# yvette256/nerfstudio-thermal

Measured on AMD Instinct MI355X. Metric: train rays/sec (4096-ray batch, 96 samples/ray), higher is better.
Workload: dtype f32; 1 GPU; thermal-nerfacto density_mode=shared train step (pixel sampling+raygen+fwd+losses+bwd+allreduce+Adam), 4096 rays/GPU, 256/96 proposal + 48 field samples, hash 16x2^19x2 + 2x(5x2^17x2), 8 cameras (4 RGB + 4 thermal); rays_per_gpu=4096, parallelism=dp1, grad_scaler=device-side (optim.DeviceGradScaler)

## Files before the change

nerfstudio-thermal_amd/csrc/tn_field.hip:

```cpp
#include "tn_common.h"
#include "tn_field_dpos.h"
#include <stdlib.h>

typedef float f32x16 __attribute__((ext_vector_type(16)));
typedef float v4f_t __attribute__((ext_vector_type(4)));
#ifndef FRAG_NT
#define FRAG_NT 1
#endif

#define TILE 32
#define FRAG 64

__host__ __device__ __forceinline__ constexpr int RROW(int r, int h) { return (r & 3) + 8 * (r >> 2) + 4 * h; }

struct LayerGeom { int mo, ti; };
__host__ __device__ __forceinline__ constexpr int layer_mo(int l) { return (l == 0 || l == 2 || l == 3) ? 2 : 1; }
__host__ __device__ __forceinline__ constexpr int layer_ti(int l) { return l == 0 ? 1 : 2; }
__host__ __device__ __forceinline__ constexpr int layer_frags(int l) { return layer_mo(l) * layer_ti(l) * 16; }
__host__ __device__ __forceinline__ constexpr int fwd_off(int l) {
  int o = 0;
  for (int i = 0; i < l; ++i) o += layer_frags(i) * FRAG;
  return o;
}
#define PACK_FWD_FLOATS (fwd_off(5))
// ... 116 lines not shown
  int64_t bytes;
};
static inline FieldWs ws_layout(void* base, int64_t P, int training) {
  FieldWs w;
  char* p = reinterpret_cast<char*>(base);
  int64_t off = 0;
  auto take = [&](int64_t floats) {
    float* r = reinterpret_cast<float*>(p + off);
    off += ((floats * 4 + 255) / 256) * 256;
    return r;
  };
  const int64_t PT = tn_cdiv(P, 32) * 32;
  w.PT = PT;
  w.pack = take(PACK_REGION_FLOATS);
  w.pos = take(P * 4);
  w.enc = take(PT * 32);
  w.sel = take(P);
  w.sh = take(P * 16);
  if (training) {
    w.h1 = take(PT * 64); w.hin = take(PT * 16); w.hh1 = take(PT * 64); w.hh2 = take(PT * 64); w.y = take(P * 4);
    w.g_enc = take(P * 32);
    w.jac = take(PT * 96);
    w.cam_bias = take((int64_t)FIELD_MAX_IMAGES * 64 + 64);
    w.scatter = take(tn_scatter_scratch_bytes(P, TN_MAX_LEVELS) / 4);
  } else {
    w.h1 = w.hin = w.hh1 = w.hh2 = w.y = w.g_enc = w.jac = w.cam_bias = nullptr;
    w.scatter = nullptr;
  }
  w.bytes = off;
  return w;
}
extern "C" int64_t tn_field_workspace_bytes(int64_t num_points, int32_t training) {
  if (num_points < 0) return TN_EINVAL;
  return ws_layout(nullptr, num_points, training).bytes;
}

__device__ __forceinline__ void sh16(float dx, float dy, float dz, float* c);
template <bool PACK>
__global__ void __launch_bounds__(256) k_field_prep(FieldK f, float* __restrict__ pack, const float* __restrict__ origins,
                                                    const float* __restrict__ directions, const float* __restrict__ e_bins, int64_t N, int S,
                                                    float4* __restrict__ pos, float* __restrict__ sel, float* __restrict__ shtab,
                                                    float4* __restrict__ zero, int64_t zero_n4, float4* __restrict__ cam_bias, int cam_bias_n4) {
  int bid = blockIdx.x, nblk = gridDim.x;
  if (PACK) {
    const int pkb = PACK_BLOCKS + ((f.num_images < FIELD_MAX_IMAGES ? f.num_images : FIELD_MAX_IMAGES) * 64 + 255) / 256 + PACK_BF_WORDS / 256;
    if (bid < pkb) { field_pack_body(f, pack, bid * 256 + threadIdx.x); return; }
    bid -= pkb; nblk -= pkb;
  }
  for (int64_t i = bid * (int64_t)blockDim.x + threadIdx.x; i < zero_n4; i += (int64_t)nblk * blockDim.x) zero[i] = make_float4(0.f, 0.f, 0.f, 0.f);
  for (int64_t i = bid * (int64_t)blockDim.x + threadIdx.x; i < cam_bias_n4; i += (int64_t)nblk * blockDim.x) cam_bias[i] = make_float4(0.f, 0.f, 0.f, 0.f);
  if (cam_bias_n4 > 0 && bid == 0 && threadIdx.x == 0) cam_bias[FIELD_MAX_IMAGES * 16] = make_float4(0.f, 0.f, 0.f, 0.f);
  const int64_t P = N * (int64_t)S;
  for (int64_t p = bid * (int64_t)blockDim.x + threadIdx.x; p < P; p += (int64_t)nblk * blockDim.x) {
    const int64_t ray = tn_div_index(p, S, P);
    const int s = (int)(p - ray * S);
    const float* o = origins + ray * 3;
    const float* d = directions + ray * 3;
    const float* eb = e_bins + ray * (S + 1) + s;
    const Contracted c = tn_contract(o[0], o[1], o[2], d[0], d[1], d[2], eb[0], eb[1]);
    const float m = c.sel ? 1.0f : 0.0f;
    pos[p] = make_float4(c.px, c.py, c.pz, m);
    sel[p] = m;
    if (s == 0) {
      float sh[16];
      sh16(d[0], d[1], d[2], sh);
#pragma unroll
      for (int hh = 0; hh < 2; ++hh)
#pragma unroll
        for (int r = 0; r < 8; ++r) shtab[ray * 16 + hh * 8 + r] = sh[(r & 3) + 8 * (r >> 2) + 4 * hh];
    }
  }
}

#ifndef ENC_PER
#define ENC_PER 4
#endif
#define ENC_CHUNK (128 * ENC_PER)
#define ENC_MAX_ITEMS 2
static_assert(TN_MAX_LEVELS <= 8 * ENC_MAX_ITEMS, "encode plan");
struct EncSched {
  int16_t level[8][ENC_MAX_ITEMS];
  int32_t first[8][ENC_MAX_ITEMS + 1];
  int32_t c0[8][ENC_MAX_ITEMS];
  int32_t blocks_per_xcd;
};
static EncSched make_enc_sched(const TnGrid& g, int64_t P) {
  EncSched sc;
  const int chunks = (int)tn_cdiv(P, ENC_CHUNK);
  int mx = 0;
  for (int x = 0; x < 8; ++x) {
    int n = 0;
    sc.first[x][0] = 0;
    for (int l = x; l < g.num_levels && n < ENC_MAX_ITEMS; l += 8) {
      sc.level[x][n] = (int16_t)l;
      sc.c0[x][n] = 0;
      sc.first[x][n + 1] = sc.first[x][n] + chunks;
      ++n;
    }
    for (int i = n; i < ENC_MAX_ITEMS; ++i) { sc.level[x][i] = -1; sc.c0[x][i] = 0; sc.first[x][i + 1] = sc.first[x][n]; }
    mx = sc.first[x][n] > mx ? sc.first[x][n] : mx;
  }
  sc.blocks_per_xcd = mx;
  return sc;
}
template <bool JAC>
__global__ void __launch_bounds__(256) k_field_encode_xcd(GridK g, EncSched sc, const float4* __restrict__ pos, int64_t P, int64_t PT,
                                                          float* __restrict__ enc, float* __restrict__ jac) {
  const int x = blockIdx.x & 7, q = blockIdx.x >> 3;
  int item = 0;
#pragma unroll
  for (int i = 1; i < ENC_MAX_ITEMS; ++i) item += (q >= sc.first[x][i]) ? 1 : 0;
  if (q >= sc.first[x][ENC_MAX_ITEMS]) return;
  const int l = sc.level[x][item];
  const int chunk = sc.c0[x][item] + (q - sc.first[x][item]);
  const float res = g.res[l];
  const uint32_t off = (uint32_t)l * g.tsize;
  const int side = threadIdx.x & 1;
  const int64_t base = (int64_t)chunk * ENC_CHUNK + (threadIdx.x >> 1);
  float2 fv[ENC_PER][4];
  float ox[ENC_PER], oy[ENC_PER], oz[ENC_PER];
#pragma unroll
  for (int u = 0; u < ENC_PER; ++u) {
    int64_t p = base + u * 128;
    if (p >= P) p = P - 1;
    const float4 c = pos[p];
    const float sx = c.x * res, sy = c.y * res, sz = c.z * res;
    const float fxf = floorf(sx), fyf = floorf(sy), fzf = floorf(sz);
    const uint32_t xi = side ? (uint32_t)(int)fxf : (uint32_t)(int)ceilf(sx);
    const uint32_t hcy = (uint32_t)(int)ceilf(sy) * TN_PRIME_Y, hfy = (uint32_t)(int)fyf * TN_PRIME_Y;
    const uint32_t hcz = (uint32_t)(int)ceilf(sz) * TN_PRIME_Z, hfz = (uint32_t)(int)fzf * TN_PRIME_Z;
    ox[u] = sx - fxf; oy[u] = sy - fyf; oz[u] = sz - fzf;
    fv[u][0] = tn_table_entry(g.table, ((xi ^ hcy ^ hcz) & g.mask) + off);
    fv[u][1] = tn_table_entry(g.table, ((xi ^ hfy ^ hcz) & g.mask) + off);
    fv[u][2] = tn_table_entry(g.table, ((xi ^ hcy ^ hfz) & g.mask) + off);
    fv[u][3] = tn_table_entry(g.table, ((xi ^ hfy ^ hfz) & g.mask) + off);
  }
#pragma unroll
  for (int u = 0; u < ENC_PER; ++u) {
    const int64_t p = base + u * 128;
    const float ux = 1.0f - ox[u], uy = 1.0f - oy[u], uz = 1.0f - oz[u];
    const float wk = side ? ux : ox[u], wr = side ? ox[u] : ux;
    float t[4], dk[4];
#pragma unroll
    for (int k = 0; k < 4; ++k) {
      const float keep = side ? fv[u][k].y : fv[u][k].x, send = side ? fv[u][k].x : fv[u][k].y;
      const float recv = __int_as_float(__builtin_amdgcn_mov_dpp(__float_as_int(send), 0xB1, 0xF, 0xF, true));
      t[k] = keep * wk + recv * wr;
      if (JAC) dk[k] = side ? recv - keep : keep - recv;
    }
    const float f0312 = t[0] * oy[u] + t[1] * uy, f4756 = t[2] * oy[u] + t[3] * uy;
    const float r = f0312 * oz[u] + f4756 * uz;
    if (p >= P) continue;
    enc[((int64_t)l * PT + p) * 2 + side] = r;
    if (JAC) {
      const float dx = (dk[0] * oy[u] + dk[1] * uy) * oz[u] + (dk[2] * oy[u] + dk[3] * uy) * uz;
      const float dy = (t[0] - t[1]) * oz[u] + (t[2] - t[3]) * uz;
      const float dz = f0312 - f4756;
      float* jp = jac + ((int64_t)l * 3 * PT + p) * 2 + side;
      __builtin_nontemporal_store(dx * res, jp);
      __builtin_nontemporal_store(dy * res, jp + 2 * PT);
      __builtin_nontemporal_store(dz * res, jp + 4 * PT);
    }
  }
}

__global__ void __launch_bounds__(256) k_field_emb_finish(float* __restrict__ cam_bias, uint32_t* __restrict__ counter, const float* __restrict__ hw0,
                                                          const float* __restrict__ emb, float* __restrict__ gemb, float* __restrict__ ghw0, int num_images) {
  __shared__ float sums[64];
  __shared__ int flag;
  emb_finish_jobs(cam_bias, counter, hw0, emb, gemb, ghw0, num_images, sums, &flag, blockIdx.x, gridDim.x);
}

__global__ void __launch_bounds__(256) k_field_dpos(DposArgs a) {
  __shared__ float emb_sums[64];
  __shared__ int emb_flag;
  field_dpos_body(a, blockIdx.x, gridDim.x, emb_sums, &emb_flag);
}

__device__ __forceinline__ void sh16(float dx, float dy, float dz, float* c) {
  float x = (dx + 1.0f) / 2.0f, y = (dy + 1.0f) / 2.0f, z = (dz + 1.0f) / 2.0f;
  float xx = x * x, yy = y * y, zz = z * z;
  c[0] = 0.28209479177387814f;
  c[1] = 0.4886025119029199f * y;
  c[2] = 0.4886025119029199f * z;
  c[3] = 0.4886025119029199f * x;
  c[4] = 1.0925484305920792f * x * y;
  c[5] = 1.0925484305920792f * y * z;
  c[6] = 0.9461746957575601f * zz - 0.31539156525251999f;
  c[7] = 1.0925484305920792f * x * z;
  c[8] = 0.5462742152960396f * (xx - yy);
  c[9] = 0.5900435899266435f * y * (3.0f * xx - yy);
  c[10] = 2.890611442640554f * x * y * z;
  c[11] = 0.4570457994644658f * y * (5.0f * zz - 1.0f);
  c[12] = 0.3731763325901154f * z * (5.0f * zz - 3.0f);
  c[13] = 0.4570457994644658f * x * (5.0f * zz - 1.0f);
  c[14] = 1.445305721320277f * z * (xx - yy);
  c[15] = 0.5900435899266435f * x * (xx - 3.0f * yy);
}

#define MFMA(a, b, c) __builtin_amdgcn_mfma_f32_32x32x2f32((a), (b), (c), 0, 0, 0)
typedef __bf16 bf16x8 __attribute__((ext_vector_type(8)));
#define MFMAB(a, b, c) __builtin_amdgcn_mfma_f32_32x32x16_bf16((a), (b), (c), 0, 0, 0)
template <int S8>
__device__ __forceinline__ void bf_split8(const f32x16& v, bf16x8& hi, bf16x8& lo) {
#pragma unroll
  for (int q = 0; q < 8; ++q) {
    const float x = v[8 * S8 + q];
    const __bf16 hq = (__bf16)x;
    hi[q] = hq;
    lo[q] = (__bf16)(x - (float)hq);
  }
}
template <int T>
__device__ __forceinline__ void bf3_tile_fwd(const float* __restrict__ frags, int lane, const f32x16& x, f32x16& o0, f32x16& o1) {
  bf16x8 bh, bl;
#define BF_FRAG(m, s, part) (*reinterpret_cast<const bf16x8*>(frags + ((((((m) * 2 + T) * 2 + (s)) * 2 + (part))) << 8) + (lane << 2)))
#define BF_KSTEP(s)                                                                       \
  {                                                                                       \
    const bf16x8 a0h = BF_FRAG(0, s, 0), a0l = BF_FRAG(0, s, 1), a1h = BF_FRAG(1, s, 0), a1l = BF_FRAG(1, s, 1); \
    o0 = MFMAB(a0l, bh, o0); o1 = MFMAB(a1l, bh, o1);                                     \
    o0 = MFMAB(a0h, bl, o0); o1 = MFMAB(a1h, bl, o1);                                     \
    o0 = MFMAB(a0h, bh, o0); o1 = MFMAB(a1h, bh, o1);                                     \
  }
  bf_split8<0>(x, bh, bl);
  BF_KSTEP(0)
  bf_split8<1>(x, bh, bl);
  BF_KSTEP(1)
#undef BF_KSTEP
#undef BF_FRAG
}

__device__ __forceinline__ f32x16 bias_tile(const float* __restrict__ lds_bias, int layer, int m, int h) {
  f32x16 v;
#pragma unroll
  for (int r = 0; r < 16; ++r) v[r] = lds_bias[layer * 64 + 32 * m + RROW(r, h)];
  return v;
}
__device__ __forceinline__ f32x16 relu16(f32x16 v) {
#pragma unroll
  for (int r = 0; r < 16; ++r) v[r] = fmaxf(v[r], 0.0f);
  return v;
}
__device__ __forceinline__ void store_tile(float* __restrict__ base, int64_t p, int ld, int m, int h, const f32x16& v) {
#pragma unroll
  for (int g = 0; g < 4; ++g)
    *reinterpret_cast<float4*>(base + p * ld + 32 * m + 8 * g + 4 * h) = make_float4(v[4 * g], v[4 * g + 1], v[4 * g + 2], v[4 * g + 3]);
}
__device__ __forceinline__ f32x16 load_tile(const float* __restrict__ base, int64_t p, int ld, int m, int h) {
  f32x16 v;
#pragma unroll
  for (int g = 0; g < 4; ++g) {
    float4 t = *reinterpret_cast<const float4*>(base + p * ld + 32 * m + 8 * g + 4 * h);
    v[4 * g] = t.x; v[4 * g + 1] = t.y; v[4 * g + 2] = t.z; v[4 * g + 3] = t.w;
  }
  return v;
}

__device__ __forceinline__ void store_frag(float* __restrict__ base, int64_t tile, int M, int m, int lane, const f32x16& v) {
  v4f_t* b = reinterpret_cast<v4f_t*>(base) + ((tile * M + m) * 4) * 64 + lane;
#pragma unroll
  for (int g = 0; g < 4; ++g) {
    const v4f_t t = {v[4 * g], v[4 * g + 1], v[4 * g + 2], v[4 * g + 3]};
    if (FRAG_NT) __builtin_nontemporal_store(t, b + g * 64); else b[g * 64] = t;
  }
}
__device__ __forceinline__ f32x16 load_frag(const float* __restrict__ base, int64_t tile, int M, int m, int lane) {
  const v4f_t* b = reinterpret_cast<const v4f_t*>(base) + ((tile * M + m) * 4) * 64 + lane;
  f32x16 v;
#pragma unroll
  for (int g = 0; g < 4; ++g) {
    const v4f_t t = FRAG_NT ? __builtin_nontemporal_load(b + g * 64) : b[g * 64];
    v[4 * g] = t.x; v[4 * g + 1] = t.y; v[4 * g + 2] = t.z; v[4 * g + 3] = t.w;
  }
  return v;
}
__device__ __forceinline__ void store_bo(float* __restrict__ base, int64_t tile, int lane, const f32x16& bo) {
  v4f_t* b = reinterpret_cast<v4f_t*>(base) + tile * 128 + lane;
  const v4f_t t0 = {bo[0], bo[1], bo[2], bo[3]}, t1 = {bo[4], bo[5], bo[6], bo[7]};
  if (FRAG_NT) { __builtin_nontemporal_store(t0, b); __builtin_nontemporal_store(t1, b + 64); }
  else { b[0] = t0; b[64] = t1; }
}
__device__ __forceinline__ int64_t hin_logit_index(int64_t tile, int j) { return (tile * 128 + j) * 4; }
__device__ __forceinline__ f32x16 load_enc_lm(const float* __restrict__ enc, int64_t PT, int64_t pc, int h, int L) {
  f32x16 v;
  const uint32_t voff = (uint32_t)(((int64_t)(2 * h) * PT + pc) * 8);
  const char* e = reinterpret_cast<const char*>(enc);
#pragma unroll
  for (int q = 0; q < 4; ++q) {
    const int l0 = 4 * q + 2 * h;
    const char* b0 = e + (int64_t)(4 * q) * PT * 8;
    const float2 a = l0 < L ? *reinterpret_cast<const float2*>(b0 + voff) : make_float2(0.f, 0.f);
    const float2 b = l0 + 1 < L ? *reinterpret_cast<const float2*>(b0 + PT * 8 + voff) : make_float2(0.f, 0.f);
    v[4 * q] = a.x; v[4 * q + 1] = a.y; v[4 * q + 2] = b.x; v[4 * q + 3] = b.y;
  }
  return v;
}

#ifndef FWD_THREADS
#define FWD_THREADS 256
#endif
#ifndef FWD_ABLATE
#define FWD_ABLATE 0
#endif
#ifndef FWD_HEAD2_MFMA
#define FWD_HEAD2_MFMA 0
#endif
#ifndef FWD_EMB_MFMA
#define FWD_EMB_MFMA 0
#endif
template <bool TRAIN, bool BF3>
__global__ void __launch_bounds__(FWD_THREADS, FWD_THREADS / 128) k_field_mlp_fwd(const float* __restrict__ pack, const float* __restrict__ encs, int L,
                                                            int64_t PT, const float* __restrict__ sels, const float* __restrict__ shtab,
                                                            const int64_t* __restrict__ cam_idx, const float* __restrict__ emb, int num_images,
                                                            int use_cam_emb, int64_t N, int S, int C, float* __restrict__ density,
                                                            float* __restrict__ rgb, float* __restrict__ density_pre, float* __restrict__ h1s,
                                                            float* __restrict__ hins, float* __restrict__ hh1s, float* __restrict__ hh2s,
                                                            float* __restrict__ ys) {
  extern __shared__ __attribute__((aligned(16))) float lds[];
  const int lane = threadIdx.x & 63, j = lane & 31, h = lane >> 5;
  const int64_t P = N * (int64_t)S;
  const int64_t ntiles = tn_cdiv(P, TILE);
  const int64_t wave = (int64_t)blockIdx.x * (blockDim.x >> 6) + (threadIdx.x >> 6);
  const int64_t nwaves = (int64_t)gridDim.x * (blockDim.x >> 6);
  f32x16 nin;
  if (wave < ntiles) {
    const int64_t p0 = wave * TILE + j;
    nin = (FWD_ABLATE & 4) ? f32x16{0.1f, 0.2f, 0.3f, 0.4f, 0.5f, 0.6f, 0.7f, 0.8f, 0.1f, 0.2f, 0.3f, 0.4f, 0.5f, 0.6f, 0.7f, 0.8f} : load_enc_lm(encs, PT, p0 < P ? p0 : P - 1, h, L);
  }
  for (int i = threadIdx.x * 4; i < PACK_FWD_TOTAL; i += blockDim.x * 4) {
    const float* src = (BF3 && i >= fwd_off(2) && i < fwd_off(4)) ? pack + PACK_BF_OFF + (i - fwd_off(2)) : pack + i;
    *reinterpret_cast<float4*>(lds + i) = *reinterpret_cast<const float4*>(src);
  }
  __syncthreads();
  const float* lbias = lds + PACK_BIAS_OFF;
#define AF(layer, m, t, r) lds[fwd_off(layer) + ((((m) * layer_ti(layer) + (t)) * 16 + (r)) << 6) + lane]
  for (int64_t tile = wave; tile < ntiles; tile += nwaves) {
    const int64_t p = tile * TILE + j;
    const bool valid = p < P;
    const int64_t pc = valid ? p : P - 1;
    const int64_t ray = tn_div_index(pc, S, P);
    const float sl = sels[pc];
    const f32x16 in0 = nin;
    f32x16 a0 = bias_tile(lbias, 0, 0, h), a1 = bias_tile(lbias, 0, 1, h);
#pragma unroll
    for (int r = 0; r < 16; ++r) {
      a0 = MFMA(AF(0, 0, 0, r), in0[r], a0);
      a1 = MFMA(AF(0, 1, 0, r), in0[r], a1);
    }
    {
      const int64_t tn = tile + nwaves < ntiles ? tile + nwaves : tile;
      const int64_t pn = tn * TILE + j;
      if (!(FWD_ABLATE & 4)) nin = load_enc_lm(encs, PT, pn < P ? pn : P - 1, h, L);
    }
    __builtin_amdgcn_sched_barrier(0);
    a0 = relu16(a0); a1 = relu16(a1);
    if (TRAIN && !(FWD_ABLATE & 1)) { store_frag(h1s, tile, 2, 0, lane, a0); store_frag(h1s, tile, 2, 1, lane, a1); }
    f32x16 bo = bias_tile(lbias, 1, 0, h);
#pragma unroll
    for (int r = 0; r < 16; ++r) bo = MFMA(AF(1, 0, 0, r), a0[r], bo);
#pragma unroll
    for (int r = 0; r < 16; ++r) bo = MFMA(AF(1, 0, 1, r), a1[r], bo);
    __builtin_amdgcn_sched_barrier(0);
    if (valid && h == 0 && !(FWD_ABLATE & 16)) {
      float pre = bo[0];
      density[p] = expf(pre) * sl;
      if (density_pre) density_pre[p] = pre;
    }
    if (TRAIN && !(FWD_ABLATE & 1)) store_bo(hins, tile, lane, bo);
    f32x16 hi0, hi1;
    {
      const float4 zz = make_float4(0.1f, 0.2f, 0.3f, 0.4f);
      const float4 s0 = (FWD_ABLATE & 2) ? zz : *reinterpret_cast<const float4*>(shtab + ray * 16 + h * 8), s1 = (FWD_ABLATE & 2) ? zz : *reinterpret_cast<const float4*>(shtab + ray * 16 + h * 8 + 4);
      hi0[0] = s0.x; hi0[1] = s0.y; hi0[2] = s0.z; hi0[3] = s0.w; hi0[4] = s1.x; hi0[5] = s1.y; hi0[6] = s1.z; hi0[7] = s1.w;
    }
#pragma unroll
    for (int r = 0; r < 8; ++r) hi0[8 + r] = bo[r];
    f32x16 c0 = bias_tile(lbias, 2, 0, h), c1 = bias_tile(lbias, 2, 1, h);
    constexpr bool CAMHEAD = TRAIN && !FWD_EMB_MFMA;
    if (CAMHEAD && !(FWD_ABLATE & 2)) {
      int64_t cam = cam_idx[ray];
      if (cam < 0 || cam >= num_images) cam = 0;
      const float* chp = pack + PACK_CAMHEAD_OFF + cam * 64 + 4 * h;
#pragma unroll
      for (int gq = 0; gq < 4; ++gq) {
        const float4 u0 = *reinterpret_cast<const float4*>(chp + 8 * gq), u1 = *reinterpret_cast<const float4*>(chp + 32 + 8 * gq);
        c0[4 * gq] += u0.x; c0[4 * gq + 1] += u0.y; c0[4 * gq + 2] += u0.z; c0[4 * gq + 3] += u0.w;
        c1[4 * gq] += u1.x; c1[4 * gq + 1] += u1.y; c1[4 * gq + 2] += u1.z; c1[4 * gq + 3] += u1.w;
      }
    } else if (!CAMHEAD) {
      const float* ebp;
      if (use_cam_emb) {
        int64_t cam = cam_idx[ray];
        if (cam < 0 || cam >= num_images) cam = 0;
        ebp = emb + cam * 32;
      } else {
        ebp = lds + PACK_MEANEMB_OFF;
      }
#pragma unroll
      for (int gq = 0; gq < 4; ++gq)
#pragma unroll
        for (int q = 0; q < 4; ++q) hi1[4 * gq + q] = ebp[8 * gq + 4 * h + q];
    }
    __builtin_amdgcn_sched_barrier(0);
    if (BF3) {
      bf3_tile_fwd<0>(lds + fwd_off(2), lane, hi0, c0, c1);
      if (!CAMHEAD && !(FWD_ABLATE & 2)) bf3_tile_fwd<1>(lds + fwd_off(2), lane, hi1, c0, c1);
    } else {
#pragma unroll
      for (int r = 0; r < 16; ++r) { c0 = MFMA(AF(2, 0, 0, r), hi0[r], c0); c1 = MFMA(AF(2, 1, 0, r), hi0[r], c1); }
      if (!CAMHEAD && !(FWD_ABLATE & 2)) {
#pragma unroll
        for (int r = 0; r < 16; ++r) { c0 = MFMA(AF(2, 0, 1, r), hi1[r], c0); c1 = MFMA(AF(2, 1, 1, r), hi1[r], c1); }
      }
    }
    __builtin_amdgcn_sched_barrier(0);
    c0 = relu16(c0); c1 = relu16(c1);
    if (TRAIN && !(FWD_ABLATE & 1)) { store_frag(hh1s, tile, 2, 0, lane, c0); store_frag(hh1s, tile, 2, 1, lane, c1); }
    f32x16 d0 = bias_tile(lbias, 3, 0, h), d1 = bias_tile(lbias, 3, 1, h);
    if (BF3) {
      bf3_tile_fwd<0>(lds + fwd_off(2) + PACK_BF_LAYER_WORDS, lane, c0, d0, d1);
      bf3_tile_fwd<1>(lds + fwd_off(2) + PACK_BF_LAYER_WORDS, lane, c1, d0, d1);
    } else {
#pragma unroll
      for (int r = 0; r < 16; ++r) { d0 = MFMA(AF(3, 0, 0, r), c0[r], d0); d1 = MFMA(AF(3, 1, 0, r), c0[r], d1); }
#pragma unroll
      for (int r = 0; r < 16; ++r) { d0 = MFMA(AF(3, 0, 1, r), c1[r], d0); d1 = MFMA(AF(3, 1, 1, r), c1[r], d1); }
    }
    __builtin_amdgcn_sched_barrier(0);
    d0 = relu16(d0); d1 = relu16(d1);
    if (TRAIN && !(FWD_ABLATE & 1)) { store_frag(hh2s, tile, 2, 0, lane, d0); store_frag(hh2s, tile, 2, 1, lane, d1); }
    __builtin_amdgcn_sched_barrier(0);
    float e[4] = {0.f, 0.f, 0.f, 0.f};
    if (FWD_ABLATE & 8) { if (d0[0] + d1[5] == 1.2345e-30f) rgb[p] = d0[3]; continue; }
#if FWD_HEAD2_MFMA
    {
      f32x16 em = bias_tile(lbias, 4, 0, h);
#pragma unroll
      for (int r = 0; r < 16; ++r) em = MFMA(AF(4, 0, 0, r), d0[r], em);
#pragma unroll
      for (int r = 0; r < 16; ++r) em = MFMA(AF(4, 0, 1, r), d1[r], em);
      e[0] = em[0]; e[1] = em[1]; e[2] = em[2]; e[3] = em[3];
    }
#else
    {
      const float* w4 = lds + fwd_off(4) + 32 * h;
#pragma unroll
      for (int r = 0; r < 16; ++r) {
        const float4 wa = *reinterpret_cast<const float4*>(w4 + (r << 6)), wb = *reinterpret_cast<const float4*>(w4 + ((16 + r) << 6));
        e[0] = fmaf(wa.x, d0[r], e[0]); e[1] = fmaf(wa.y, d0[r], e[1]); e[2] = fmaf(wa.z, d0[r], e[2]); e[3] = fmaf(wa.w, d0[r], e[3]);
        e[0] = fmaf(wb.x, d1[r], e[0]); e[1] = fmaf(wb.y, d1[r], e[1]); e[2] = fmaf(wb.z, d1[r], e[2]); e[3] = fmaf(wb.w, d1[r], e[3]);
      }
#pragma unroll
      for (int cc = 0; cc < 4; ++cc) e[cc] = (e[cc] + __shfl_xor(e[cc], 32, 64)) + lbias[4 * 64 + cc];
    }
#endif
    if (valid && h == 0) {
      float y[4] = {0.f, 0.f, 0.f, 0.f};
#pragma unroll
      for (int cc = 0; cc < 4; ++cc)
        if (cc < C) { y[cc] = 1.0f / (1.0f + expf(-e[cc])); rgb[p * C + cc] = y[cc]; }
      if (TRAIN) *reinterpret_cast<float4*>(ys + p * 4) = make_float4(y[0], y[1], y[2], y[3]);
    }
  }
#undef AF
}

template <bool TRAIN>
__global__ void __launch_bounds__(256, 2) k_field_density_only(const float* __restrict__ pack, const float* __restrict__ enc, int L, int64_t PT,
                                                               const float* __restrict__ sel, int64_t P, float* __restrict__ density,
                                                               float* __restrict__ h1s, float* __restrict__ hins) {
  extern __shared__ __attribute__((aligned(16))) float lds[];
  for (int i = threadIdx.x * 4; i < PACK_FWD_TOTAL; i += blockDim.x * 4)
    *reinterpret_cast<float4*>(lds + i) = *reinterpret_cast<const float4*>(pack + i);
  __syncthreads();
  const float* lbias = lds + PACK_BIAS_OFF;
  const int lane = threadIdx.x & 63, j = lane & 31, h = lane >> 5;
  const int64_t ntiles = tn_cdiv(P, TILE);
  const int64_t wave = (int64_t)blockIdx.x * (blockDim.x >> 6) + (threadIdx.x >> 6);
  const int64_t nwaves = (int64_t)gridDim.x * (blockDim.x >> 6);
#define AF(layer, m, t, r) lds[fwd_off(layer) + ((((m) * layer_ti(layer) + (t)) * 16 + (r)) << 6) + lane]
  for (int64_t tile = wave; tile < ntiles; tile += nwaves) {
    int64_t p = tile * TILE + j;
    bool valid = p < P;
    int64_t pc = valid ? p : P - 1;
    f32x16 in0 = load_enc_lm(enc, PT, pc, h, L);
    f32x16 a0 = bias_tile(lbias, 0, 0, h), a1 = bias_tile(lbias, 0, 1, h);
#pragma unroll
    for (int r = 0; r < 16; ++r) { a0 = MFMA(AF(0, 0, 0, r), in0[r], a0); a1 = MFMA(AF(0, 1, 0, r), in0[r], a1); }
    a0 = relu16(a0); a1 = relu16(a1);
    if (TRAIN) { store_frag(h1s, tile, 2, 0, lane, a0); store_frag(h1s, tile, 2, 1, lane, a1); }
    f32x16 bo = bias_tile(lbias, 1, 0, h);
#pragma unroll
    for (int r = 0; r < 16; ++r) bo = MFMA(AF(1, 0, 0, r), a0[r], bo);
#pragma unroll
    for (int r = 0; r < 16; ++r) bo = MFMA(AF(1, 0, 1, r), a1[r], bo);
    if (valid && h == 0) {
      density[p] = expf(bo[0]) * sel[p];
      if (TRAIN) hins[hin_logit_index(tile, j)] = bo[0];
    }
  }
#undef AF
}

#define TSTR 68
#define FB_TILE_FLOATS (32 * TSTR)
#define FB_WAVE_FLOATS (2 * FB_TILE_FLOATS + 128 + 32)
#define FB_LDS_FLOATS (PACK_BWD_FLOATS + 4 * FB_WAVE_FLOATS)
#define FB_RED_W3 0
#define FB_RED_W2 4096
#define FB_RED_A_TOTAL 6144
#define FB_RED_W0 0
#define FB_RED_W4 2048
#define FB_RED_W1 3072
#define FB_RED_B3 4096
#define FB_RED_B2 4160
#define FB_RED_B0 4224
#define FB_RED_B4 4288
#define FB_RED_B1 4304
#define FB_RED_B_TOTAL 4320
#define FB_EMB_MERGE_FLOATS (4 * 64 + 8)
static_assert(4 * FB_RED_A_TOTAL + FB_EMB_MERGE_FLOATS <= FB_LDS_FLOATS && FB_RED_B_TOTAL <= FB_RED_A_TOTAL, "four copies of a block-sum pass (+ the embedding merge) must fit in LDS");
typedef float f32x4v __attribute__((ext_vector_type(4)));
#define MFMA16(a, b, c) __builtin_amdgcn_mfma_f32_16x16x4f32((a), (b), (c), 0, 0, 0)
#define WAVE_LDS_SYNC()                                   \
  do {                                                    \
    __builtin_amdgcn_fence(__ATOMIC_RELEASE, "wavefront"); \
    __builtin_amdgcn_wave_barrier();                      \
    __builtin_amdgcn_fence(__ATOMIC_ACQUIRE, "wavefront"); \
  } while (0)

__device__ __forceinline__ void lds_put_tile(float* __restrict__ buf, int j, int h, int m, const f32x16& v) {
#pragma unroll
  for (int g = 0; g < 4; ++g)
    *reinterpret_cast<float4*>(buf + j * TSTR + 32 * m + 8 * g + 4 * h) = make_float4(v[4 * g], v[4 * g + 1], v[4 * g + 2], v[4 * g + 3]);
}
template <int MO, int MI>
__device__ __forceinline__ void wgrad_tile32(const float* __restrict__ bufY, const float* __restrict__ bufX, int j, int h, f32x16 (&acc)[MO][MI],
                                             float (&bsum)[MO]) {
#pragma unroll
  for (int t = 0; t < 16; ++t) {
    float av[MO], bv[MI];
#pragma unroll
    for (int a = 0; a < MO; ++a) av[a] = bufY[(2 * t + h) * TSTR + 32 * a + j];
#pragma unroll
    for (int b = 0; b < MI; ++b) bv[b] = bufX[(2 * t + h) * TSTR + 32 * b + j];
#pragma unroll
    for (int a = 0; a < MO; ++a) {
      bsum[a] += av[a];
#pragma unroll
      for (int b = 0; b < MI; ++b) acc[a][b] = MFMA(av[a], bv[b], acc[a][b]);
    }
  }
}
__device__ __forceinline__ void wgrad_tile16(const float* __restrict__ bufY, int ldy, int ncols, const float* __restrict__ bufX, int lane,
                                             f32x4v (&acc)[4], float& bsum) {
  const int c = lane & 15, ks = lane >> 4;
#pragma unroll
  for (int t = 0; t < 8; ++t) {
    const float av = c < ncols ? bufY[(4 * t + ks) * ldy + c] : 0.0f;
    bsum += av;
#pragma unroll
    for (int b = 0; b < 4; ++b) acc[b] = MFMA16(av, bufX[(4 * t + ks) * TSTR + 16 * b + c], acc[b]);
  }
}

template <int M>
__device__ __forceinline__ void bf3_tile_one(const float* __restrict__ frags, int lane, const f32x16& x, f32x16& o) {
  bf16x8 bh, bl;
#define BF_FRAG(s, part) (*reinterpret_cast<const bf16x8*>(frags + ((((M * 2 + (s)) * 2 + (part))) << 8) + (lane << 2)))
  bf_split8<0>(x, bh, bl);
  { const bf16x8 ah = BF_FRAG(0, 0), al = BF_FRAG(0, 1); o = MFMAB(al, bh, o); o = MFMAB(ah, bl, o); o = MFMAB(ah, bh, o); }
  bf_split8<1>(x, bh, bl);
  { const bf16x8 ah = BF_FRAG(1, 0), al = BF_FRAG(1, 1); o = MFMAB(al, bh, o); o = MFMAB(ah, bl, o); o = MFMAB(ah, bh, o); }
#undef BF_FRAG
}
template <int MO, int MI>
__device__ __forceinline__ void wgrad_tile32_bf3(const float* __restrict__ bufY, const float* __restrict__ bufX, int j, int h, f32x16 (&acc)[MO][MI],
                                                 float (&bsum)[MO]) {
#pragma unroll
  for (int s = 0; s < 2; ++s) {
    bf16x8 ah[MO], al[MO], bh[MI], bl[MI];
#pragma unroll
    for (int a = 0; a < MO; ++a) {
#pragma unroll
      for (int q = 0; q < 8; ++q) {
        const float x = bufY[(16 * s + 8 * h + q) * TSTR + 32 * a + j];
        bsum[a] += x;
        const __bf16 hq = (__bf16)x;
        ah[a][q] = hq;
        al[a][q] = (__bf16)(x - (float)hq);
      }
    }
#pragma unroll
    for (int b = 0; b < MI; ++b) {
#pragma unroll
      for (int q = 0; q < 8; ++q) {
        const float x = bufX[(16 * s + 8 * h + q) * TSTR + 32 * b + j];
        const __bf16 hq = (__bf16)x;
        bh[b][q] = hq;
        bl[b][q] = (__bf16)(x - (float)hq);
      }
    }
#pragma unroll
    for (int a = 0; a < MO; ++a)
#pragma unroll
      for (int b = 0; b < MI; ++b) {
        acc[a][b] = MFMAB(al[a], bh[b], acc[a][b]);
        acc[a][b] = MFMAB(ah[a], bl[b], acc[a][b]);
        acc[a][b] = MFMAB(ah[a], bh[b], acc[a][b]);
      }
  }
}

struct FusedGrads {
  float *gw0, *gb0, *gw1, *gb1, *ghw0, *ghb0, *ghw1, *ghb1, *ghw2, *ghb2, *gemb;
};

#ifndef FB_ABLATE
#define FB_ABLATE 0
#endif
struct FbSmall {
  float pre_logit, g_dens, sel_p;
  float g3[4];
  int cam;
  int ray;
};
template <bool DENS_ONLY>
__device__ __forceinline__ FbSmall fb_load_small(int64_t tile, int64_t tile_addr, int j, int h, int64_t P, int S, int C, int num_images,
                                                 const float* __restrict__ hins, const float* __restrict__ d_density, const float* __restrict__ sel,
                                                 const float* __restrict__ ys, const float* __restrict__ d_rgb, const int64_t* __restrict__ cam_idx) {
  FbSmall q;
  const int64_t p = tile * TILE + j;
  const bool valid = p < P;
  const int64_t pc = valid ? p : P - 1;
  q.pre_logit = hins[hin_logit_index(tile_addr, j)];
  q.g_dens = valid ? d_density[pc] : 0.0f;
  q.sel_p = sel[pc];
  q.g3[0] = q.g3[1] = q.g3[2] = q.g3[3] = 0.0f;
  q.cam = -1;
  q.ray = 0;
  if (!DENS_ONLY) {
    q.ray = (int)tn_div_index(pc, S, P);
    const int64_t cam = cam_idx[q.ray];
    q.cam = valid ? ((cam < 0 || cam >= num_images) ? 0 : (int)cam) : -1;
    if (valid && h == 0) {
      const float4 y4 = *reinterpret_cast<const float4*>(ys + p * 4);
      const float yv[4] = {y4.x, y4.y, y4.z, y4.w};
#pragma unroll
      for (int c = 0; c < 4; ++c)
        if (c < C) q.g3[c] = d_rgb[p * C + c] * yv[c] * (1.0f - yv[c]);
    }
  }
  return q;
}

#ifndef FB_NO_SB
#define FB_NO_SB 0
#endif
#ifndef FB_TOUCH
#define FB_TOUCH 0
#endif
#define FB_SB() do { if (!FB_NO_SB) __builtin_amdgcn_sched_barrier(0); } while (0)
template <bool DENS_ONLY, bool BF3>
__global__ void __launch_bounds__(256, 1) k_field_bwd_fused(const float* __restrict__ pack, const float* __restrict__ sel, const float* __restrict__ ys,
                                                            const float* __restrict__ d_rgb, const float* __restrict__ d_density,
                                                            const int64_t* __restrict__ cam_idx, int num_images, int64_t P, int S, int C,
                                                            const float* __restrict__ shtab, const float* __restrict__ emb,
                                                            float* __restrict__ cam_bias, int L, int64_t PT,
                                                            const float* __restrict__ encs, const float* __restrict__ h1s,
                                                            const float* __restrict__ hins, const float* __restrict__ hh1s,
                                                            const float* __restrict__ hh2s, float* __restrict__ g_enc, FusedGrads G,
                                                            uint32_t* __restrict__ zero_ptr, int zero_words) {
  extern __shared__ __attribute__((aligned(16))) float lds[];
  tn_zero_words(zero_ptr, zero_words);
  const float* src = pack + PACK_BWD_OFF;
  constexpr int PACK_TRIPS = PACK_BWD_FLOATS / (256 * 4);
  static_assert(PACK_BWD_FLOATS % (256 * 4) == 0, "the packed backward fragments are copied in whole trips of 256 threads x float4");
  float4 wq[PACK_TRIPS];
#pragma unroll
  for (int k = 0; k < PACK_TRIPS; ++k) {
    const int i = (k * 256 + (int)threadIdx.x) * 4;
    const float* sp = (BF3 && i >= fwd_off(2) && i < fwd_off(4)) ? pack + PACK_BF_BWD_OFF + (i - fwd_off(2)) : src + i;
    wq[k] = *reinterpret_cast<const float4*>(sp);
  }
  const int lane = threadIdx.x & 63, j = lane & 31, h = lane >> 5, wv = threadIdx.x >> 6;
  float* bufY = lds + PACK_BWD_FLOATS + wv * FB_WAVE_FLOATS;
  float* bufX = bufY + FB_TILE_FLOATS;
  float* bufG = bufX + FB_TILE_FLOATS;
  int* bufC = reinterpret_cast<int*>(bufG + 128);
  const int64_t ntiles = tn_cdiv(P, TILE);
  const int64_t wave = (int64_t)blockIdx.x * 4 + wv;
  const int64_t nwaves = (int64_t)gridDim.x * 4;
#define AB(layer, t, m, r) lds[fwd_off(layer) + ((((t) * layer_mo(layer) + (m)) * 16 + (r)) << 6) + lane]
  const f32x16 zero16 = {0, 0, 0, 0, 0, 0, 0, 0, 0, 0, 0, 0, 0, 0, 0, 0};
  const f32x4v zero4 = {0, 0, 0, 0};
  f32x16 acc3[2][2], acc2[2][1], acc0[2][1];
  f32x4v acc4[4], acc1[4];
  float bs3[2] = {0.f, 0.f}, bs2[2] = {0.f, 0.f}, bs0[2] = {0.f, 0.f}, bs4 = 0.f, bs1 = 0.f;
#pragma unroll
  for (int a = 0; a < 2; ++a) {
    acc0[a][0] = zero16;
    acc2[a][0] = zero16;
#pragma unroll
    for (int b = 0; b < 2; ++b) acc3[a][b] = zero16;
  }
#pragma unroll
  for (int b = 0; b < 4; ++b) { acc4[b] = zero4; acc1[b] = zero4; }
  int emb_cam = -1;
  float emb_sum = 0.0f;
  const int64_t tpw = tn_cdiv(ntiles, nwaves);
  const int64_t tile_begin = wave * tpw;
  const int64_t tile_end = (wave + 1) * tpw < ntiles ? (wave + 1) * tpw : ntiles;
  f32x16 nx0 = zero16, nx1 = zero16;
  FbSmall nsm;
  if (tile_begin < tile_end) {
    nsm = fb_load_small<DENS_ONLY>(tile_begin, tile_begin, j, h, P, S, C, num_images, hins, d_density, sel, ys, d_rgb, cam_idx);
    nx0 = load_frag(DENS_ONLY ? h1s : hh2s, tile_begin, 2, 0, lane);
    nx1 = load_frag(DENS_ONLY ? h1s : hh2s, tile_begin, 2, 1, lane);
  }
  float touch_acc = 0.0f;
#pragma unroll
  for (int k = 0; k < PACK_TRIPS; ++k) *reinterpret_cast<float4*>(lds + (k * 256 + (int)threadIdx.x) * 4) = wq[k];
  __syncthreads();
  for (int64_t tile = tile_begin; tile < tile_end; ++tile) {
    const int64_t p = tile * TILE + j;
    const bool valid = p < P;
    const int64_t pc = valid ? p : P - 1;
    const FbSmall sm = nsm;
    float tch0 = 0.0f, tch1 = 0.0f, tch2 = 0.0f;
    if (FB_TOUCH && tile + 1 < tile_end) {
      const int64_t tn = tile + 1;
      if (!DENS_ONLY) tch0 = hh1s[(tn * 2 * 4 * 64) * 4 + lane * 32];
      tch1 = h1s[(tn * 2 * 4 * 64) * 4 + lane * 32];
      if (lane < 16) {
        if (!DENS_ONLY) tch2 = hins[(tn * 128) * 4 + lane * 32];
      } else if (lane < 48) {
        const int l = (lane - 16) >> 1;
        if (l < L) tch2 = encs[((int64_t)l * PT + tn * TILE) * 2 + ((lane - 16) & 1) * 32];
      }
    }
    f32x16 di0 = zero16;
    f32x16 s0, s1;
    if (!DENS_ONLY) {
      if (h == 0) {
        *reinterpret_cast<float4*>(bufG + j * 4) = make_float4(sm.g3[0], sm.g3[1], sm.g3[2], sm.g3[3]);
        bufC[j] = sm.cam;
      }
      f32x16 dd0 = zero16, dd1 = zero16;
#pragma unroll
      for (int r = 0; r < 4; ++r) { dd0 = MFMA(AB(4, 0, 0, r), sm.g3[r], dd0); dd1 = MFMA(AB(4, 1, 0, r), sm.g3[r], dd1); }
      f32x16 t0 = load_frag(hh1s, tile, 2, 0, lane), t1 = load_frag(hh1s, tile, 2, 1, lane);
#pragma unroll
      for (int r = 0; r < 16; ++r) { dd0[r] = nx0[r] > 0.0f ? dd0[r] : 0.0f; dd1[r] = nx1[r] > 0.0f ? dd1[r] : 0.0f; }
      lds_put_tile(bufX, j, h, 0, nx0); lds_put_tile(bufX, j, h, 1, nx1);
      lds_put_tile(bufY, j, h, 0, dd0); lds_put_tile(bufY, j, h, 1, dd1);
      WAVE_LDS_SYNC();
      if (!(FB_ABLATE & 4)) wgrad_tile16(bufG, 4, C, bufX, lane, acc4, bs4);
      FB_SB();
      f32x16 dc0 = zero16, dc1 = zero16;
      if (BF3) {
        bf3_tile_fwd<0>(lds + fwd_off(2) + PACK_BF_LAYER_WORDS, lane, dd0, dc0, dc1);
        bf3_tile_fwd<1>(lds + fwd_off(2) + PACK_BF_LAYER_WORDS, lane, dd1, dc0, dc1);
      } else {
#pragma unroll
        for (int r = 0; r < 16; ++r) { dc0 = MFMA(AB(3, 0, 0, r), dd0[r], dc0); dc1 = MFMA(AB(3, 1, 0, r), dd0[r], dc1); }
#pragma unroll
        for (int r = 0; r < 16; ++r) { dc0 = MFMA(AB(3, 0, 1, r), dd1[r], dc0); dc1 = MFMA(AB(3, 1, 1, r), dd1[r], dc1); }
      }
      FB_SB();
      WAVE_LDS_SYNC();
#pragma unroll
      for (int r = 0; r < 16; ++r) { dc0[r] = t0[r] > 0.0f ? dc0[r] : 0.0f; dc1[r] = t1[r] > 0.0f ? dc1[r] : 0.0f; }
      lds_put_tile(bufX, j, h, 0, t0); lds_put_tile(bufX, j, h, 1, t1);
      const v4f_t* bp = reinterpret_cast<const v4f_t*>(hins) + tile * 128 + lane;
      const v4f_t hb0 = FRAG_NT ? __builtin_nontemporal_load(bp) : bp[0], hb1 = FRAG_NT ? __builtin_nontemporal_load(bp + 64) : bp[64];
      WAVE_LDS_SYNC();
      if (!(FB_ABLATE & 2)) {
        if (BF3) wgrad_tile32_bf3<2, 2>(bufY, bufX, j, h, acc3, bs3); else wgrad_tile32<2, 2>(bufY, bufX, j, h, acc3, bs3);
      }
      FB_SB();
      WAVE_LDS_SYNC();
      {
        const float* shp = shtab + (int64_t)sm.ray * 16 + h * 8;
        const float4 sa = *reinterpret_cast<const float4*>(shp), sb = *reinterpret_cast<const float4*>(shp + 4);
        lds_put_tile(bufY, j, h, 0, dc0); lds_put_tile(bufY, j, h, 1, dc1);
        t0[0] = sa.x; t0[1] = sa.y; t0[2] = sa.z; t0[3] = sa.w; t0[4] = sb.x; t0[5] = sb.y; t0[6] = sb.z; t0[7] = sb.w;
        t0[8] = hb0.x; t0[9] = hb0.y; t0[10] = hb0.z; t0[11] = hb0.w; t0[12] = hb1.x; t0[13] = hb1.y; t0[14] = hb1.z; t0[15] = hb1.w;
      }
      lds_put_tile(bufX, j, h, 0, t0);
      s0 = load_frag(h1s, tile, 2, 0, lane); s1 = load_frag(h1s, tile, 2, 1, lane);
      WAVE_LDS_SYNC();
// ... 509 lines not shown
```

Before: 6.258 million rays/s.

## Prefetch per-tile side inputs and batch weight staging loads in field MLP kernels

The forward field MLP kernel now prefetches the next tile's selector, SH table entries, camera index and camera-head bias one iteration ahead, and keeps them in registers alongside the existing encoding prefetch. Weight staging into LDS is split into a batch of global loads followed by LDS stores, so the camera-head prefetch can be issued in between. The density-only kernel gets the same staging helper plus software-pipelined encoding loads. The goal is to hide global-memory latency behind MFMA work, at the cost of higher register pressure and possible occupancy loss.

```diff
diff --git a/nerfstudio-thermal_amd/csrc/tn_field.hip b/nerfstudio-thermal_amd/csrc/tn_field.hip
--- a/nerfstudio-thermal_amd/csrc/tn_field.hip
+++ b/nerfstudio-thermal_amd/csrc/tn_field.hip
@@ -442,6 +442,27 @@
 #ifndef FWD_ABLATE
 #define FWD_ABLATE 0
 #endif
+template <bool BF3, int THREADS, typename F>
+__device__ __forceinline__ void stage_pack_fwd(const float* __restrict__ pack, float* __restrict__ lds, F between) {
+  constexpr int N4 = PACK_FWD_TOTAL / 4, TRIPS = (N4 + THREADS - 1) / THREADS;
+  static_assert(PACK_FWD_TOTAL % 4 == 0 && fwd_off(2) % 4 == 0 && fwd_off(4) % 4 == 0, "pack layout");
+  if (FWD_ABLATE & 32) { between(); return; }
+  float4 w[TRIPS];
+#pragma unroll
+  for (int k = 0; k < TRIPS; ++k) {
+    int i = (k * THREADS + (int)threadIdx.x) * 4;
+    if ((k + 1) * THREADS > N4 && i >= PACK_FWD_TOTAL) i = PACK_FWD_TOTAL - 4;
+    const float* src = (BF3 && i >= fwd_off(2) && i < fwd_off(4)) ? pack + PACK_BF_OFF + (i - fwd_off(2)) : pack + i;
+    w[k] = *reinterpret_cast<const float4*>(src);
+  }
+  between();
+#pragma unroll
+  for (int k = 0; k < TRIPS; ++k) {
+    const int i = (k * THREADS + (int)threadIdx.x) * 4;
+    if ((k + 1) * THREADS <= N4 || i < PACK_FWD_TOTAL) *reinterpret_cast<float4*>(lds + i) = w[k];
+  }
+  __syncthreads();
+}
 #ifndef FWD_HEAD2_MFMA
 #define FWD_HEAD2_MFMA 0
 #endif
@@ -462,24 +483,49 @@
   const int64_t ntiles = tn_cdiv(P, TILE);
   const int64_t wave = (int64_t)blockIdx.x * (blockDim.x >> 6) + (threadIdx.x >> 6);
   const int64_t nwaves = (int64_t)gridDim.x * (blockDim.x >> 6);
+  constexpr bool CAMHEAD = TRAIN && !FWD_EMB_MFMA;
   f32x16 nin;
-  if (wave < ntiles) {
-    const int64_t p0 = wave * TILE + j;
-    nin = (FWD_ABLATE & 4) ? f32x16{0.1f, 0.2f, 0.3f, 0.4f, 0.5f, 0.6f, 0.7f, 0.8f, 0.1f, 0.2f, 0.3f, 0.4f, 0.5f, 0.6f, 0.7f, 0.8f} : load_enc_lm(encs, PT, p0 < P ? p0 : P - 1, h, L);
-  }
-  for (int i = threadIdx.x * 4; i < PACK_FWD_TOTAL; i += blockDim.x * 4) {
-    const float* src = (BF3 && i >= fwd_off(2) && i < fwd_off(4)) ? pack + PACK_BF_OFF + (i - fwd_off(2)) : pack + i;
-    *reinterpret_cast<float4*>(lds + i) = *reinterpret_cast<const float4*>(src);
-  }
-  __syncthreads();
+  float nsl = 0.0f;
+  float4 ns0 = make_float4(0.1f, 0.2f, 0.3f, 0.4f), ns1 = ns0, nch[8];
+  int64_t ncam = 0;
+  auto request_tile = [&](int64_t t) {
+    if (FWD_ABLATE & 64) t = wave & 63;
+    const int64_t pn = t * TILE + j;
+    const int64_t pcn = pn < P ? pn : P - 1;
+    const int64_t rayn = tn_div_index(pcn, S, P);
+    if (!(FWD_ABLATE & 4)) nin = load_enc_lm(encs, PT, pcn, h, L);
+    nsl = sels[pcn];
+    if (!(FWD_ABLATE & 2)) {
+      ns0 = *reinterpret_cast<const float4*>(shtab + rayn * 16 + h * 8);
+      ns1 = *reinterpret_cast<const float4*>(shtab + rayn * 16 + h * 8 + 4);
+      if (CAMHEAD) ncam = cam_idx[rayn];
+    }
+    return rayn;
+  };
+  auto request_camhead = [&]() {
+    if (CAMHEAD && !(FWD_ABLATE & 2)) {
+      int64_t cam = ncam;
+      if (cam < 0 || cam >= num_images) cam = 0;
+      const float* chp = pack + PACK_CAMHEAD_OFF + cam * 64 + 4 * h;
+#pragma unroll
+      for (int gq = 0; gq < 4; ++gq) {
+        nch[gq] = *reinterpret_cast<const float4*>(chp + 8 * gq);
+        nch[4 + gq] = *reinterpret_cast<const float4*>(chp + 32 + 8 * gq);
+      }
+    }
+  };
+  int64_t nray = 0;
+  if (FWD_ABLATE & 4) nin = f32x16{0.1f, 0.2f, 0.3f, 0.4f, 0.5f, 0.6f, 0.7f, 0.8f, 0.1f, 0.2f, 0.3f, 0.4f, 0.5f, 0.6f, 0.7f, 0.8f};
+  if (wave < ntiles) nray = request_tile(wave);
+  stage_pack_fwd<BF3, FWD_THREADS>(pack, lds, [&]() { if (wave < ntiles) request_camhead(); });
   const float* lbias = lds + PACK_BIAS_OFF;
 #define AF(layer, m, t, r) lds[fwd_off(layer) + ((((m) * layer_ti(layer) + (t)) * 16 + (r)) << 6) + lane]
   for (int64_t tile = wave; tile < ntiles; tile += nwaves) {
     const int64_t p = tile * TILE + j;
     const bool valid = p < P;
-    const int64_t pc = valid ? p : P - 1;
-    const int64_t ray = tn_div_index(pc, S, P);
-    const float sl = sels[pc];
+    const int64_t ray = nray;
+    const float sl = nsl;
+    const float4 s0 = ns0, s1 = ns1;
     const f32x16 in0 = nin;
     f32x16 a0 = bias_tile(lbias, 0, 0, h), a1 = bias_tile(lbias, 0, 1, h);
 #pragma unroll
@@ -487,11 +533,7 @@
       a0 = MFMA(AF(0, 0, 0, r), in0[r], a0);
       a1 = MFMA(AF(0, 1, 0, r), in0[r], a1);
     }
-    {
-      const int64_t tn = tile + nwaves < ntiles ? tile + nwaves : tile;
-      const int64_t pn = tn * TILE + j;
-      if (!(FWD_ABLATE & 4)) nin = load_enc_lm(encs, PT, pn < P ? pn : P - 1, h, L);
-    }
+    nray = request_tile(tile + nwaves < ntiles ? tile + nwaves : tile);
     __builtin_amdgcn_sched_barrier(0);
     a0 = relu16(a0); a1 = relu16(a1);
     if (TRAIN && !(FWD_ABLATE & 1)) { store_frag(h1s, tile, 2, 0, lane, a0); store_frag(h1s, tile, 2, 1, lane, a1); }
@@ -508,22 +550,14 @@
     }
     if (TRAIN && !(FWD_ABLATE & 1)) store_bo(hins, tile, lane, bo);
     f32x16 hi0, hi1;
-    {
-      const float4 zz = make_float4(0.1f, 0.2f, 0.3f, 0.4f);
-      const float4 s0 = (FWD_ABLATE & 2) ? zz : *reinterpret_cast<const float4*>(shtab + ray * 16 + h * 8), s1 = (FWD_ABLATE & 2) ? zz : *reinterpret_cast<const float4*>(shtab + ray * 16 + h * 8 + 4);
-      hi0[0] = s0.x; hi0[1] = s0.y; hi0[2] = s0.z; hi0[3] = s0.w; hi0[4] = s1.x; hi0[5] = s1.y; hi0[6] = s1.z; hi0[7] = s1.w;
-    }
+    hi0[0] = s0.x; hi0[1] = s0.y; hi0[2] = s0.z; hi0[3] = s0.w; hi0[4] = s1.x; hi0[5] = s1.y; hi0[6] = s1.z; hi0[7] = s1.w;
 #pragma unroll
     for (int r = 0; r < 8; ++r) hi0[8 + r] = bo[r];
     f32x16 c0 = bias_tile(lbias, 2, 0, h), c1 = bias_tile(lbias, 2, 1, h);
-    constexpr bool CAMHEAD = TRAIN && !FWD_EMB_MFMA;
     if (CAMHEAD && !(FWD_ABLATE & 2)) {
-      int64_t cam = cam_idx[ray];
-      if (cam < 0 || cam >= num_images) cam = 0;
-      const float* chp = pack + PACK_CAMHEAD_OFF + cam * 64 + 4 * h;
 #pragma unroll
       for (int gq = 0; gq < 4; ++gq) {
-        const float4 u0 = *reinterpret_cast<const float4*>(chp + 8 * gq), u1 = *reinterpret_cast<const float4*>(chp + 32 + 8 * gq);
+        const float4 u0 = nch[gq], u1 = nch[4 + gq];
         c0[4 * gq] += u0.x; c0[4 * gq + 1] += u0.y; c0[4 * gq + 2] += u0.z; c0[4 * gq + 3] += u0.w;
         c1[4 * gq] += u1.x; c1[4 * gq + 1] += u1.y; c1[4 * gq + 2] += u1.z; c1[4 * gq + 3] += u1.w;
       }
@@ -553,6 +587,7 @@
         for (int r = 0; r < 16; ++r) { c0 = MFMA(AF(2, 0, 1, r), hi1[r], c0); c1 = MFMA(AF(2, 1, 1, r), hi1[r], c1); }
       }
     }
+    request_camhead();
     __builtin_amdgcn_sched_barrier(0);
     c0 = relu16(c0); c1 = relu16(c1);
     if (TRAIN && !(FWD_ABLATE & 1)) { store_frag(hh1s, tile, 2, 0, lane, c0); store_frag(hh1s, tile, 2, 1, lane, c1); }
@@ -610,23 +645,29 @@
                                                                const float* __restrict__ sel, int64_t P, float* __restrict__ density,
                                                                float* __restrict__ h1s, float* __restrict__ hins) {
   extern __shared__ __attribute__((aligned(16))) float lds[];
-  for (int i = threadIdx.x * 4; i < PACK_FWD_TOTAL; i += blockDim.x * 4)
-    *reinterpret_cast<float4*>(lds + i) = *reinterpret_cast<const float4*>(pack + i);
-  __syncthreads();
-  const float* lbias = lds + PACK_BIAS_OFF;
   const int lane = threadIdx.x & 63, j = lane & 31, h = lane >> 5;
   const int64_t ntiles = tn_cdiv(P, TILE);
   const int64_t wave = (int64_t)blockIdx.x * (blockDim.x >> 6) + (threadIdx.x >> 6);
   const int64_t nwaves = (int64_t)gridDim.x * (blockDim.x >> 6);
+  f32x16 nin;
+  if (wave < ntiles) {
+    const int64_t p0 = wave * TILE + j;
+    nin = load_enc_lm(enc, PT, p0 < P ? p0 : P - 1, h, L);
+  }
+  stage_pack_fwd<false, 256>(pack, lds, []() {});
+  const float* lbias = lds + PACK_BIAS_OFF;
 #define AF(layer, m, t, r) lds[fwd_off(layer) + ((((m) * layer_ti(layer) + (t)) * 16 + (r)) << 6) + lane]
   for (int64_t tile = wave; tile < ntiles; tile += nwaves) {
     int64_t p = tile * TILE + j;
     bool valid = p < P;
-    int64_t pc = valid ? p : P - 1;
-    f32x16 in0 = load_enc_lm(enc, PT, pc, h, L);
+    const f32x16 in0 = nin;
     f32x16 a0 = bias_tile(lbias, 0, 0, h), a1 = bias_tile(lbias, 0, 1, h);
 #pragma unroll
     for (int r = 0; r < 16; ++r) { a0 = MFMA(AF(0, 0, 0, r), in0[r], a0); a1 = MFMA(AF(0, 1, 0, r), in0[r], a1); }
+    {
+      const int64_t pn = (tile + nwaves < ntiles ? tile + nwaves : tile) * TILE + j;
+      nin = load_enc_lm(enc, PT, pn < P ? pn : P - 1, h, L);
+    }
     a0 = relu16(a0); a1 = relu16(a1);
     if (TRAIN) { store_frag(h1s, tile, 2, 0, lane, a0); store_frag(h1s, tile, 2, 1, lane, a1); }
     f32x16 bo = bias_tile(lbias, 1, 0, h);
```

New measurement: 6.289 million rays/s (median of 6 runs). No clear change (+0.5%).
